# fanzhongyi/ExploreMultiModal

Hardware: AMD Instinct MI355X
Metric: image-text pairs/sec fwd+bwd, VLMo-Base, 1/2/4/8 MI355X; % bf16 MFMA roofline (higher is better)
Workload: dtype bf16

## Files before the change

### exploremultimodal_amd/csrc/attention.hip

```cpp
#include "common.h"
#include "vlmo_hip.h"

namespace {

struct AttnArgs {
    const bf16* qkv;
    const bf16* ctx;
    const bf16* dctx;
    bf16* out;
    float* lse;
    float* qvsum;
    const int32_t* seg;
    const int32_t* keymask;
    int lse_stride, heads, d;
    float scale, scale_log2e;
    uint32_t drop_thresh, drop_cmp;
    float inv_keep;
    uint64_t seed;
    int bh0;
};

#define LOG2E 1.4426950408889634f
#define LN2 0.6931471805599453f

// ... 216 lines not shown
    const bool active = w < nq;
    const int qi = w * 32 + l31;
    const int qrow = sr.row(qi);
    bf16x8 qf[4];
    if (active) {
        const bf16* qp = a.qkv + (size_t)qrow * ld + hd * 64 + 8 * h;
#pragma unroll
        for (int s = 0; s < 4; ++s) qf[s] = *(const bf16x8*)(qp + 16 * s);
    }
    const int ninstr = FRINGE ? min(nq * 4, NPAD >> 3) : nq * 4;
    for (int ii = w; ii < ninstr; ii += nw) {
        const int chhi = lane >> 5, rowlo = (lane >> 2) & 7, pc = lane & 3;
        const int row = ii * 8 + rowlo;
        const int ch = chhi * 4 + (pc ^ ((row >> 2) & 3));
        const size_t r = (size_t)sr.row(row);
        glds16(a.qkv + r * ld + a.d + hd * 64 + ch * 8, Kimg + ii * 1024);
        glds16(a.qkv + r * ld + 2 * a.d + hd * 64 + ch * 8, Vimg + ii * 1024);
    }
    if (FRINGE && nq == 9 && w < 4) {
        const int chhi = lane >> 5, rowlo = (lane >> 2) & 7, pc = lane & 3;
        const int row = w * 8 + rowlo;
        const int ch = chhi * 4 + (pc ^ ((row >> 2) & 3));
        glds16(a.qkv + (size_t)sr.row(256 + row) * ld + hd * 64 + ch * 8, Pbuf + w * 1024);
    }
    for (int i = threadIdx.x; i < (FRINGE ? 288 : NPAD); i += blockDim.x) {
        kbias[i] = key_bias(a.keymask, sr.row(i), i, N);
    }
    asm volatile("s_waitcnt vmcnt(0)" ::: "memory");
    __syncthreads();
    if (!active) return;

    const int xq = (l31 >> 2) & 3;
    const int rf0 = 1024 * (l31 >> 3) + 64 * (l31 & 7) + 16 * (h ^ xq);
    const int rf1 = 1024 * (l31 >> 3) + 64 * (l31 & 7) + 16 * ((2 + h) ^ xq);
    const int tg = (lane >> 4) & 1, tq = (lane >> 2) & 3, tp = lane & 3;
    const int trl = 64 * (4 * h + tq) + 16 * ((2 * tg + (tp >> 1)) ^ h) + 8 * (tp & 1);
    const int trh = 1024 + 64 * (4 * h + tq) + 16 * ((2 * tg + (tp >> 1)) ^ ((2 + h) & 3)) + 8 * (tp & 1);
    auto rfrag = [&](const char* img_rb, int s) -> bf16x8 {
        return *(const bf16x8*)(img_rb + 512 * (s >> 1) + ((s & 1) ? rf1 : rf0));
    };
    auto tfrag = [&](const char* img_rb, int dt) -> bf16x8 {
        const bf16x4 lo = lds_tr4<bf16>(img_rb + 512 * dt + trl);
        const bf16x4 hi = lds_tr4<bf16>(img_rb + 512 * dt + trh);
        return bf16x8{lo[0], lo[1], lo[2], lo[3], hi[0], hi[1], hi[2], hi[3]};
    };
    auto other_half = [&](float v) -> float {
        const uint32_t u = __builtin_bit_cast(uint32_t, v);
        const auto r = __builtin_amdgcn_permlane32_swap(u, u, false, false);
        return __builtin_bit_cast(float, h ? r[0] : r[1]);
    };
    auto s_tile = [&](int kt) -> f32x16 {
        f32x16 acc;
        const float* kb = kbias + kt * 32 + 4 * h;
#pragma unroll
        for (int g4 = 0; g4 < 4; ++g4) {
            const f32x4 v = *(const f32x4*)(kb + 8 * g4);
#pragma unroll
            for (int e = 0; e < 4; ++e) acc[4 * g4 + e] = v[e];
        }
        const char* kimg = Kimg + 4096 * kt;
#pragma unroll
        for (int s = 0; s < 4; ++s) acc = Elem<bf16>::mfma(rfrag(kimg, s), qf[s], acc);
        return acc;
    };

    const uint32_t akey = att_key(a.seed, bh + a.bh0);
    const uint32_t rq = ((uint32_t)qi * 512u + 4u * h) * ATT_G + akey;
    const float c2 = a.scale_log2e;
    const float thr = 8.f / c2;
    float m_run = -INFINITY;
    f32x2 l2 = {0.f, 0.f};
    f32x16 O[2] = {zero16(), zero16()};
    auto consume = [&](f32x16& S, int kt) {
        float mx = fmaxf(fmaxf(S[0], S[1]), S[2]);
#pragma unroll
        for (int i = 3; i < 15; i += 2) mx = fmaxf(fmaxf(mx, S[i]), S[i + 1]);
        mx = fmaxf(mx, S[15]);
        mx = fmaxf(mx, other_half(mx));
        if (__builtin_amdgcn_ballot_w64(mx - m_run > thr)) {
            asm volatile("" ::: "memory");
            const float m_new = fmaxf(m_run, mx);
            const float alpha = (m_run == -INFINITY) ? 1.f : __builtin_amdgcn_exp2f((m_run - m_new) * c2);
            l2 *= alpha;
#pragma unroll
            for (int dt = 0; dt < 2; ++dt)
#pragma unroll
                for (int i = 0; i < 16; ++i) O[dt][i] *= alpha;
            m_run = m_new;
        }
        const float msub = (m_run == -INFINITY) ? 0.f : -m_run * c2;
        const f32x2 c2v = {c2, c2}, msv = {msub, msub};
#pragma unroll
        for (int i = 0; i < 16; i += 2) {
            const f32x2 t = f32x2{S[i], S[i + 1]} * c2v + msv;
            const f32x2 pr = {__builtin_amdgcn_exp2f(t[0]), __builtin_amdgcn_exp2f(t[1])};
            l2 += pr;
            S[i] = pr[0];
            S[i + 1] = pr[1];
        }
        if (a.drop_thresh) S = drop_tile(S, rq + (uint32_t)(kt * 32) * ATT_G, a.drop_cmp);
        const char* vimg = Vimg + 4096 * kt;
#pragma unroll
        for (int s2 = 0; s2 < 2; ++s2) {
            bf16x8 pf;
#pragma unroll
            for (int j = 0; j < 8; ++j) pf[j] = (bf16)S[8 * s2 + j];
#pragma unroll
            for (int dt = 0; dt < 2; ++dt) O[dt] = Elem<bf16>::mfma(tfrag(vimg + 2048 * s2, dt), pf, O[dt]);
        }
    };
    f32x16 S0 = s_tile(0), S1;
    for (int kt = 0; kt < nq; kt += 2) {
        if (kt + 1 < nq) S1 = s_tile(kt + 1);
        __builtin_amdgcn_sched_barrier(0);
        consume(S0, kt);
        __builtin_amdgcn_sched_barrier(0);
        if (kt + 1 < nq) {
            if (kt + 2 < nq) S0 = s_tile(kt + 2);
            __builtin_amdgcn_sched_barrier(0);
            consume(S1, kt + 1);
            __builtin_amdgcn_sched_barrier(0);
        }
    }
    const float l_run = l2[0] + l2[1];
    const float l_tot = l_run + other_half(l_run);
    if (qi < N) store_ctx(a, O, l_tot, (m_run * c2 + log2f(l_tot)) * LN2, bh, hd, qi, qrow, h);

    if constexpr (FRINGE) {
        if (nq < 9) return;
        float* fmax = kbias + 288;
        float* fsum = fmax + 288;
        bf16x8 qF[4];
#pragma unroll
        for (int s = 0; s < 4; ++s) qF[s] = rfrag(Pbuf, s);
        auto s_fringe = [&](int kt) -> f32x16 {
            f32x16 acc;
            const float* kb = kbias + kt * 32 + 4 * h;
#pragma unroll
            for (int g4 = 0; g4 < 4; ++g4) {
                const f32x4 v = *(const f32x4*)(kb + 8 * g4);
#pragma unroll
                for (int e = 0; e < 4; ++e) acc[4 * g4 + e] = v[e];
            }
            const char* kimg = Kimg + 4096 * kt;
#pragma unroll
            for (int s = 0; s < 4; ++s) acc = Elem<bf16>::mfma(rfrag(kimg, s), qF[s], acc);
            return acc;
        };
        auto tile_max = [&](const f32x16& S) -> float {
            float mx = S[0];
#pragma unroll
            for (int i = 1; i < 16; ++i) mx = fmaxf(mx, S[i]);
            return fmaxf(mx, other_half(mx));
        };
        const bool two = (w == 0);
        f32x16 SA = s_fringe(w), SB = SA;
        if (two) SB = s_fringe(8);
        {
            const float ma = tile_max(SA), mb = tile_max(SB);
            if (h == 0) {
                fmax[w * 32 + l31] = ma;
                if (two) fmax[8 * 32 + l31] = mb;
            }
        }
        __syncthreads();
        float mstar = fmax[l31];
#pragma unroll
        for (int t = 1; t < 9; ++t) mstar = fmaxf(mstar, fmax[t * 32 + l31]);
        const float msubF = (mstar == -INFINITY) ? 0.f : -mstar * c2;
        const uint32_t rqF = ((uint32_t)(256 + l31) * 512u + 4u * h) * ATT_G + akey;
        auto soft_pack = [&](f32x16& S, int kt, bf16x8 (&pf)[2]) {
            float l = 0.f;
#pragma unroll
            for (int i = 0; i < 16; ++i) {
                S[i] = __builtin_amdgcn_exp2f(fmaf(S[i], c2, msubF));
                l += S[i];
            }
            l += other_half(l);
            if (h == 0) fsum[kt * 32 + l31] = l;
            if (a.drop_thresh) S = drop_tile(S, rqF + (uint32_t)(kt * 32) * ATT_G, a.drop_cmp);
#pragma unroll
            for (int s2 = 0; s2 < 2; ++s2)
#pragma unroll
                for (int j = 0; j < 8; ++j) pf[s2][j] = (bf16)S[8 * s2 + j];
        };
        bf16x8 pA[2], pB[2];
        soft_pack(SA, w, pA);
        if (two) soft_pack(SB, 8, pB);
        const int dtF = w & 1;
        f32x16 OF = zero16();
        for (int g = 0; g < 3; ++g) {
            if (w / 3 == g) {
                *(bf16x8*)(Pbuf + (w % 3) * 2048 + lane * 16) = pA[0];
                *(bf16x8*)(Pbuf + (w % 3) * 2048 + 1024 + lane * 16) = pA[1];
            }
            if (g == 2 && two) {
                *(bf16x8*)(Pbuf + 2 * 2048 + lane * 16) = pB[0];
                *(bf16x8*)(Pbuf + 2 * 2048 + 1024 + lane * 16) = pB[1];
            }
            __syncthreads();
            if (w >= 6) {
#pragma unroll
                for (int j = 0; j < 3; ++j)
#pragma unroll
                    for (int s2 = 0; s2 < 2; ++s2) {
                        const bf16x8 pf = *(const bf16x8*)(Pbuf + j * 2048 + s2 * 1024 + lane * 16);
                        OF = Elem<bf16>::mfma(tfrag(Vimg + 4096 * (3 * g + j) + 2048 * s2, dtF), pf, OF);
                    }
            }
            if (g < 2) __syncthreads();
        }
        const int qiF = 256 + l31;
        if (w >= 6 && qiF < N) {
            float l = fsum[l31];
#pragma unroll
            for (int t = 1; t < 9; ++t) l += fsum[t * 32 + l31];
            const float inv = a.inv_keep / l;
            bf16* op = a.out + (size_t)sr.row(qiF) * a.d + hd * 64 + 4 * h + dtF * 32;
#pragma unroll
            for (int g4 = 0; g4 < 4; ++g4) {
                bf16x4 o = {(bf16)(OF[4 * g4 + 0] * inv), (bf16)(OF[4 * g4 + 1] * inv), (bf16)(OF[4 * g4 + 2] * inv),
                            (bf16)(OF[4 * g4 + 3] * inv)};
                *(bf16x4*)(op + 8 * g4) = o;
            }
            if (w == 6 && h == 0 && a.lse) a.lse[(size_t)bh * a.lse_stride + qiF] = (mstar * c2 + log2f(l)) * LN2;
        }
    }
}

__device__ __forceinline__ float half_wave_total(float v) {
    float s_ = v + dpp_mov<0x111, 0xf, 0xf>(v);
    s_ += dpp_mov<0x112, 0xf, 0xf>(v);
    s_ += dpp_mov<0x113, 0xf, 0xf>(v);
    s_ += dpp_mov<0x114, 0xf, 0xe>(s_);
    s_ += dpp_mov<0x118, 0xf, 0xc>(s_);
    s_ += dpp_mov<0x142, 0xa, 0xf>(s_);
    return s_;
}
__device__ __forceinline__ void colsum_tile(const f32x16& t, float w, float scale, float* acc, int lane) {
    const int h = lane >> 5;
#pragma unroll
    for (int r = 0; r < 16; ++r) {
        const float v = half_wave_total(t[r] * w);
        if ((lane & 31) == 31) atomicAdd(acc + (r & 3) + 8 * (r >> 2) + 4 * h, v * scale);
    }
}
__device__ __forceinline__ void colsum_tiles(const f32x16* t, float w, float scale, float* acc, int lane) {
#pragma unroll
    for (int dt = 0; dt < 2; ++dt) colsum_tile(t[dt], w, scale, acc + dt * 32, lane);
}

__device__ __forceinline__ int slot_off(int k, int q) {
    return k * 64 + ((((q >> 2) ^ (k >> 1)) & 7) << 3) + (q & 3) * 2;
}
template <bool FRINGE>
__global__ __launch_bounds__(512) void attn_bwd1_kernel(const AttnArgs a, const int NPAD) {
    const int IMG = NPAD * 128;
    extern __shared__ __attribute__((aligned(16))) char smem[];
    char* Qimg = smem;
    char* Dimg = smem + IMG;
    char* Kimg = smem + 2 * IMG;
    const int nt = NPAD >> 5;
    char* slots = smem + 3 * IMG;
    float* kbias = (float*)(slots + 2 * nt * 2048);
    float* nlq = kbias + NPAD;
    float* ndl = nlq + NPAD;
    float* csum = ndl + NPAD;
    char* V8img = (char*)(csum + 128);

    const int lane = threadIdx.x & 63;
    const int w = __builtin_amdgcn_readfirstlane(threadIdx.x >> 6);
    const int nw = blockDim.x >> 6;
    const int bh = blockIdx.x, sidx = bh / a.heads, hd = bh % a.heads;
    const int ld = 3 * a.d;
    const SeqRows sr(a.seg, sidx);
    const int N = sr.N;
    const int nq = (N + 31) >> 5;
    const int nc = FRINGE ? min(nq, 8) : nq;
    for (int ii = w; ii < nq * 4; ii += nw) {
        const int chhi = lane >> 5, rowlo = (lane >> 2) & 7, pc = lane & 3;
        const int row = ii * 8 + rowlo;
        const int ch = chhi * 4 + (pc ^ ((row >> 2) & 3));
        const size_t r = (size_t)sr.row(row);
        glds16(a.qkv + r * ld + hd * 64 + ch * 8, Qimg + ii * 1024);
        glds16(a.qkv + r * ld + a.d + hd * 64 + ch * 8, Kimg + ii * 1024);
        glds16(a.dctx + r * a.d + hd * 64 + ch * 8, Dimg + ii * 1024);
    }
    if (FRINGE && nq > 8 && w >= 4) {
        const int chhi = lane >> 5, rowlo = (lane >> 2) & 7, pc = lane & 3;
        const int row = 256 + (w - 4) * 8 + rowlo;
        const int ch = chhi * 4 + (pc ^ ((row >> 2) & 3));
        glds16(a.qkv + (size_t)sr.row(row) * ld + 2 * a.d + hd * 64 + ch * 8, V8img + (w - 4) * 1024);
    }
    const int l31 = lane & 31, h = lane >> 5;
    const bool active = w < nc;
    const int ki = w * 32 + l31;
    const int krow = sr.row(ki);
    bf16x8 vf[4];
    if (active) {
        const bf16* kp = a.qkv + (size_t)krow * ld + a.d + hd * 64 + 8 * h;
#pragma unroll
        for (int s = 0; s < 4; ++s) vf[s] = *(const bf16x8*)(kp + a.d + 16 * s);
    }
    for (int i = threadIdx.x; i < 128; i += blockDim.x) csum[i] = 0.f;
    const float keep_prob = 1.f / a.inv_keep;
    const float inv_scale = 1.f / a.scale;
    for (int i = threadIdx.x; i < NPAD; i += blockDim.x) {
        float dl = 0.f, lq = INFINITY;
        const int row = sr.row(i);
        const float kb = key_bias(a.keymask, row, i, N);
        if (i < N) {
            const size_t o = (size_t)row * a.d + hd * 64;
            bf16x8 x[8], y[8];
#pragma unroll
            for (int c = 0; c < 8; ++c) {
                x[c] = *(const bf16x8*)(a.ctx + o + 8 * c);
                y[c] = *(const bf16x8*)(a.dctx + o + 8 * c);
            }
            lq = a.lse[(size_t)bh * a.lse_stride + i];
#pragma unroll
            for (int c = 0; c < 8; ++c)
#pragma unroll
                for (int j = 0; j < 8; ++j) dl += (float)x[c][j] * (float)y[c][j];
        }
        kbias[i] = kb;
        ndl[i] = -dl * keep_prob;
        nlq[i] = -lq * inv_scale;
    }
    asm volatile("s_waitcnt vmcnt(0)" ::: "memory");
    __syncthreads();

    const uint32_t akey = att_key(a.seed, bh + a.bh0);
    const float out_scale = a.scale * a.inv_keep;
    const float c_l2 = a.scale_log2e;
    const float kb_own = kbias[min(ki, NPAD - 1)];
    const uint32_t rl_own = (uint32_t)ki * ATT_G + akey + (uint32_t)(4 * h) * ATT_G512;
    f32x16 dK[2] = {zero16(), zero16()}, dV[2] = {zero16(), zero16()}, dQ[2] = {zero16(), zero16()};

    const int xq = (l31 >> 2) & 3;
    const int rf0 = 1024 * (l31 >> 3) + 64 * (l31 & 7) + 16 * (h ^ xq);
    const int rf1 = 1024 * (l31 >> 3) + 64 * (l31 & 7) + 16 * ((2 + h) ^ xq);
    const int tg = (lane >> 4) & 1, tq = (lane >> 2) & 3, tp = lane & 3;
    const int trl = 64 * (4 * h + tq) + 16 * ((2 * tg + (tp >> 1)) ^ h) + 8 * (tp & 1);
    const int trh = 1024 + 64 * (4 * h + tq) + 16 * ((2 * tg + (tp >> 1)) ^ ((2 + h) & 3)) + 8 * (tp & 1);
    auto rfrag = [&](const char* img_rb, int s) __attribute__((always_inline)) -> bf16x8 {
        return *(const bf16x8*)(img_rb + 512 * (s >> 1) + ((s & 1) ? rf1 : rf0));
    };
    auto tfrag = [&](const char* img_rb, int dt) __attribute__((always_inline)) -> bf16x8 {
        const bf16x4 lo = lds_tr4<bf16>(img_rb + 512 * dt + trl);
        const bf16x4 hi = lds_tr4<bf16>(img_rb + 512 * dt + trh);
        return bf16x8{lo[0], lo[1], lo[2], lo[3], hi[0], hi[1], hi[2], hi[3]};
    };
    const int sw0 = slot_off(l31, 4 * h), sw1 = slot_off(l31, 8 + 4 * h);
    const int srl = slot_off(4 * h + tq, 16 * tg + 4 * tp), srh = slot_off(8 + 4 * h + tq, 16 * tg + 4 * tp);
    auto sfrag = [&](const char* slot, int s2) __attribute__((always_inline)) -> bf16x8 {
        const bf16x4 lo = lds_tr4<bf16>(slot + 1024 * s2 + srl);
        const bf16x4 hi = lds_tr4<bf16>(slot + 1024 * s2 + srh);
        return bf16x8{lo[0], lo[1], lo[2], lo[3], hi[0], hi[1], hi[2], hi[3]};
    };

    bf16x8 qa[4], da[4], pf[2], sf[2];
    f32x16 S, dP;
    auto fetch_a = [&](int qt_) __attribute__((always_inline)) {
#pragma unroll
        for (int s = 0; s < 4; ++s) {
            qa[s] = rfrag(Qimg + qt_ * 4096, s);
            da[s] = rfrag(Dimg + qt_ * 4096, s);
        }
    };
    auto qtile = [&](int t_) __attribute__((always_inline)) {
        int q_ = w + t_;
        return q_ >= nc ? q_ - nc : q_;
    };
    auto stage_sdp = [&](int qt, const char* ktile, const bf16x8 (&vfr)[4]) __attribute__((always_inline)) {
        dP = zero16();
#pragma unroll
        for (int g4 = 0; g4 < 4; ++g4) {
            const f32x4 l4 = *(const f32x4*)(nlq + qt * 32 + 8 * g4 + 4 * h);
#pragma unroll
            for (int e = 0; e < 4; ++e) S[4 * g4 + e] = l4[e];
        }
#pragma unroll
        for (int s = 0; s < 4; ++s) {
            S = Elem<bf16>::mfma(qa[s], rfrag(ktile, s), S);
            dP = Elem<bf16>::mfma(da[s], vfr[s], dP);
        }
        __builtin_amdgcn_sched_barrier(0);
    };
    auto stage_valu_dvdk = [&](int qt, char* myslot, float kb, uint32_t rl, f32x16 (&dV)[2],
                               f32x16 (&dK)[2]) __attribute__((always_inline)) {
        bf16x8 dtr[2], qtr[2];
#pragma unroll
        for (int dt = 0; dt < 2; ++dt) {
            dtr[dt] = tfrag(Dimg + qt * 4096, dt);
            qtr[dt] = tfrag(Qimg + qt * 4096, dt);
        }
        __builtin_amdgcn_sched_barrier(0);
        if (a.drop_thresh) {
            const uint32_t rqt = rl + (uint32_t)(qt * 32) * ATT_G512;
#pragma unroll
            for (int g4 = 0; g4 < 4; ++g4) {
                const f32x4 nd = *(const f32x4*)(ndl + qt * 32 + 8 * g4 + 4 * h);
#pragma unroll
                for (int e = 0; e < 4; ++e) {
                    const int i = 4 * g4 + e;
                    const float p = __builtin_amdgcn_exp2f(fmaf(S[i], c_l2, kb));
                    const bool keep = att_mix(rqt + (uint32_t)(8 * g4 + e) * ATT_G512) >= a.drop_cmp;
                    const float pd = keep ? p : 0.f;
                    pf[i >> 3][i & 7] = (bf16)pd;
                    sf[i >> 3][i & 7] = (bf16)fmaf(pd, dP[i], p * nd[e]);
                }
            }
        } else {
#pragma unroll
            for (int g4 = 0; g4 < 4; ++g4) {
                const f32x4 nd = *(const f32x4*)(ndl + qt * 32 + 8 * g4 + 4 * h);
#pragma unroll
                for (int e = 0; e < 4; ++e) {
                    const int i = 4 * g4 + e;
                    const float p = __builtin_amdgcn_exp2f(fmaf(S[i], c_l2, kb));
                    pf[i >> 3][i & 7] = (bf16)p;
                    sf[i >> 3][i & 7] = (bf16)(p * (dP[i] + nd[e]));
                }
            }
        }
#pragma unroll
        for (int s2 = 0; s2 < 2; ++s2) {
            *(bf16x4*)(myslot + (sw0 ^ (32 * s2))) = bf16x4{sf[s2][0], sf[s2][1], sf[s2][2], sf[s2][3]};
            *(bf16x4*)(myslot + (sw1 ^ (32 * s2))) = bf16x4{sf[s2][4], sf[s2][5], sf[s2][6], sf[s2][7]};
        }
        __builtin_amdgcn_sched_barrier(0);
        bf16x8 dtr1[2], qtr1[2];
#pragma unroll
        for (int dt = 0; dt < 2; ++dt) {
            dtr1[dt] = tfrag(Dimg + qt * 4096 + 2048, dt);
            qtr1[dt] = tfrag(Qimg + qt * 4096 + 2048, dt);
        }
#pragma unroll
        for (int dt = 0; dt < 2; ++dt) {
            dV[dt] = Elem<bf16>::mfma(dtr[dt], pf[0], dV[dt]);
            dK[dt] = Elem<bf16>::mfma(qtr[dt], sf[0], dK[dt]);
        }
#pragma unroll
        for (int dt = 0; dt < 2; ++dt) {
            dV[dt] = Elem<bf16>::mfma(dtr1[dt], pf[1], dV[dt]);
            dK[dt] = Elem<bf16>::mfma(qtr1[dt], sf[1], dK[dt]);
        }
        __builtin_amdgcn_sched_barrier(0);
    };
    auto stage_dq_at = [&](const char* slot, const char* ktile, int next_q) __attribute__((always_inline)) {
        bf16x8 ktr[2][2], sb[2];
#pragma unroll
        for (int s2 = 0; s2 < 2; ++s2) {
            sb[s2] = sfrag(slot, s2);
#pragma unroll
            for (int dt = 0; dt < 2; ++dt) ktr[s2][dt] = tfrag(ktile + 2048 * s2, dt);
        }
        if (next_q >= 0) fetch_a(next_q);
        __builtin_amdgcn_sched_barrier(0);
#pragma unroll
        for (int s2 = 0; s2 < 2; ++s2)
#pragma unroll
            for (int dt = 0; dt < 2; ++dt) dQ[dt] = Elem<bf16>::mfma(ktr[s2][dt], sb[s2], dQ[dt]);
        __builtin_amdgcn_sched_barrier(0);
    };
    auto stage_dq = [&](int t, int next_q) __attribute__((always_inline)) {
        int wp = w - t;
        if (wp < 0) wp += nc;
        stage_dq_at(slots + ((t & 1) * nt + wp) * 2048, Kimg + wp * 4096, next_q);
    };
    const char* kown = Kimg + w * 4096;
    auto core_sdp = [&](int qt) __attribute__((always_inline)) { stage_sdp(qt, kown, vf); };
    auto core_valu_dvdk = [&](int qt, int t) __attribute__((always_inline)) {
        stage_valu_dvdk(qt, slots + ((t & 1) * nt + w) * 2048, kb_own, rl_own, dV, dK);
    };
    if (w >= 4) __builtin_amdgcn_s_setprio(1);
    if (!active) {
        for (int t = 0; t < nc; ++t) __syncthreads();
    } else if (w < 4) {
        fetch_a(w);
        for (int t = 0; t < nc; ++t) {
            const int qt = qtile(t);
            core_sdp(qt);
            core_valu_dvdk(qt, t);
            __syncthreads();
            stage_dq(t, t + 1 < nc ? qtile(t + 1) : -1);
        }
    } else {
        fetch_a(w);
        core_sdp(w);
        for (int t = 0; t < nc; ++t) {
            core_valu_dvdk(qtile(t), t);
            if (t > 0) stage_dq(t - 1, -1);
            if (t + 1 < nc) {
                fetch_a(qtile(t + 1));
                core_sdp(qtile(t + 1));
            }
            __syncthreads();
        }
        stage_dq(nc - 1, -1);
    }
    if (FRINGE && nq > 8) {
        auto store_tile = [&](const f32x16 (&t)[2], float sc, int row, int col0) __attribute__((always_inline)) {
            bf16* op = a.out + (size_t)row * ld + col0 + hd * 64 + 4 * h;
#pragma unroll
            for (int dt = 0; dt < 2; ++dt)
#pragma unroll
                for (int g4 = 0; g4 < 4; ++g4)
                    *(bf16x4*)(op + dt * 32 + 8 * g4) =
                        bf16x4{(bf16)(t[dt][4 * g4 + 0] * sc), (bf16)(t[dt][4 * g4 + 1] * sc),
                               (bf16)(t[dt][4 * g4 + 2] * sc), (bf16)(t[dt][4 * g4 + 3] * sc)};
        };
        fetch_a(8);
        stage_sdp(8, kown, vf);
        stage_valu_dvdk(8, slots + w * 2048, kb_own, rl_own, dV, dK);
        store_tile(dK, out_scale, krow, a.d);
        store_tile(dV, a.inv_keep, krow, 2 * a.d);
        if (a.qvsum) colsum_tiles(dV, 1.f, a.inv_keep, csum + 64, lane);
        dK[0] = zero16(), dK[1] = zero16(), dV[0] = zero16(), dV[1] = zero16();
        __syncthreads();
        const int k8 = 256 + l31;
        const char* k8tile = Kimg + 8 * 4096;
        const float kb8 = kbias[k8];
        const uint32_t rl8 = (uint32_t)k8 * ATT_G + akey + (uint32_t)(4 * h) * ATT_G512;
#pragma unroll
        for (int s = 0; s < 4; ++s) vf[s] = rfrag(V8img, s);
        char* slot1 = slots + (nt + w) * 2048;
        fetch_a(w);
        stage_sdp(w, k8tile, vf);
        stage_valu_dvdk(w, slot1, kb8, rl8, dV, dK);
        stage_dq_at(slot1, k8tile, w == 0 ? 8 : -1);
        if (w == 0) {
            stage_sdp(8, k8tile, vf);
            stage_valu_dvdk(8, slots + 8 * 2048, kb8, rl8, dV, dK);
        }
        store_tile(dQ, out_scale, krow, 0);
        if (a.qvsum) colsum_tiles(dQ, 1.f, out_scale, csum, lane);
        __syncthreads();
        auto put = [&](int region) __attribute__((always_inline)) {
            f32x4* p = (f32x4*)(smem + region * 16384) + lane;
#pragma unroll
            for (int dt = 0; dt < 2; ++dt)
#pragma unroll
                for (int g4 = 0; g4 < 4; ++g4) {
                    p[(dt * 4 + g4) * 64] = f32x4{dK[dt][4 * g4], dK[dt][4 * g4 + 1], dK[dt][4 * g4 + 2], dK[dt][4 * g4 + 3]};
                    p[(8 + dt * 4 + g4) * 64] = f32x4{dV[dt][4 * g4], dV[dt][4 * g4 + 1], dV[dt][4 * g4 + 2], dV[dt][4 * g4 + 3]};
                }
        };
        auto add = [&](int region) __attribute__((always_inline)) {
            const f32x4* p = (const f32x4*)(smem + region * 16384) + lane;
#pragma unroll
            for (int dt = 0; dt < 2; ++dt)
#pragma unroll
                for (int g4 = 0; g4 < 4; ++g4) {
                    const f32x4 uk = p[(dt * 4 + g4) * 64], uv = p[(8 + dt * 4 + g4) * 64];
#pragma unroll
                    for (int e = 0; e < 4; ++e) dK[dt][4 * g4 + e] += uk[e], dV[dt][4 * g4 + e] += uv[e];
                }
        };
        const int row8 = sr.row(k8);
        const float wt8 = k8 < N ? 1.f : 0.f;
        if (w >= 4) put(w - 4);
        if (w == 4 || w == 5) {
            const int dt = w - 4;
            f32x16 acc = zero16();
            for (int k = 0; k < 9; ++k) {
                const char* slot = slots + k * 2048;
                const bf16x8 s0 = sfrag(slot, 0), s1 = sfrag(slot, 1);
                const bf16x8 k0 = tfrag(Kimg + k * 4096, dt), k1 = tfrag(Kimg + k * 4096 + 2048, dt);
                acc = Elem<bf16>::mfma(k0, s0, acc);
                acc = Elem<bf16>::mfma(k1, s1, acc);
            }
            if (k8 < N) {
                bf16* op = a.out + (size_t)row8 * ld + hd * 64 + dt * 32 + 4 * h;
#pragma unroll
                for (int g4 = 0; g4 < 4; ++g4)
                    *(bf16x4*)(op + 8 * g4) =
                        bf16x4{(bf16)(acc[4 * g4 + 0] * out_scale), (bf16)(acc[4 * g4 + 1] * out_scale),
                               (bf16)(acc[4 * g4 + 2] * out_scale), (bf16)(acc[4 * g4 + 3] * out_scale)};
            }
            if (a.qvsum) colsum_tile(acc, wt8, out_scale, csum + dt * 32, lane);
        }
        __syncthreads();
        if (w < 4) add(w);
        if (w >= 1 && w < 4) put(w);
        __syncthreads();
        if (w == 0) {
            add(1), add(2), add(3);
            if (k8 < N) {
                store_tile(dK, out_scale, row8, a.d);
                store_tile(dV, a.inv_keep, row8, 2 * a.d);
            }
            if (a.qvsum) colsum_tiles(dV, wt8, a.inv_keep, csum + 64, lane);
        }
    } else if (active && ki < N) {
        bf16* op = a.out + (size_t)krow * ld + hd * 64 + 4 * h;
#pragma unroll
        for (int dt = 0; dt < 2; ++dt)
#pragma unroll
            for (int g4 = 0; g4 < 4; ++g4) {
                bf16x4 oq = {(bf16)(dQ[dt][4 * g4 + 0] * out_scale), (bf16)(dQ[dt][4 * g4 + 1] * out_scale),
                             (bf16)(dQ[dt][4 * g4 + 2] * out_scale), (bf16)(dQ[dt][4 * g4 + 3] * out_scale)};
                bf16x4 ok = {(bf16)(dK[dt][4 * g4 + 0] * out_scale), (bf16)(dK[dt][4 * g4 + 1] * out_scale),
                             (bf16)(dK[dt][4 * g4 + 2] * out_scale), (bf16)(dK[dt][4 * g4 + 3] * out_scale)};
                bf16x4 ov = {(bf16)(dV[dt][4 * g4 + 0] * a.inv_keep), (bf16)(dV[dt][4 * g4 + 1] * a.inv_keep),
                             (bf16)(dV[dt][4 * g4 + 2] * a.inv_keep), (bf16)(dV[dt][4 * g4 + 3] * a.inv_keep)};
                *(bf16x4*)(op + dt * 32 + 8 * g4) = oq;
                *(bf16x4*)(op + a.d + dt * 32 + 8 * g4) = ok;
                *(bf16x4*)(op + 2 * a.d + dt * 32 + 8 * g4) = ov;
            }
    }
    if (a.qvsum) {
        if (active && !(FRINGE && nq > 8)) {
            const float wt = ki < N ? 1.f : 0.f;
            colsum_tiles(dQ, wt, out_scale, csum, lane);
            colsum_tiles(dV, wt, a.inv_keep, csum + 64, lane);
        }
        __syncthreads();
        for (int i = threadIdx.x; i < 128; i += blockDim.x) {
            float* dst = a.qvsum + (size_t)sidx * 2 * a.d + (i >> 6) * a.d + hd * 64 + (i & 63);
            *dst = csum[i];
        }
    }
}

#define ATT_LW 8
#define ATT_LCH 4
#define ATT_LBUF (ATT_LCH * 4096)
#define ATT_LMAX 1024
#define ATT_LDS_FWD (4 * ATT_LBUF + ATT_LMAX * 4)
#define ATT_LDS_BWD (4 * ATT_LBUF + 3 * ATT_LMAX * 4 + ATT_LW * 64 * 4)

__device__ __forceinline__ uint32_t att_stride(int N) { return N > 512 ? 1024u : 512u; }

__device__ __forceinline__ void stage_chunk(const bf16* pa, int lda, const bf16* pb, int ldb, const SeqRows& sr, int t0,
                                            int nt, char* ia, char* ib, int w, int lane) {
    const int chhi = lane >> 5, rowlo = (lane >> 2) & 7, pc = lane & 3;
    for (int ii = w; ii < nt * 4; ii += ATT_LW) {
        const int row = t0 * 32 + ii * 8 + rowlo;
        const int ch = chhi * 4 + (pc ^ ((row >> 2) & 3));
        const size_t r = (size_t)sr.row(row);
        glds16(pa + r * lda + ch * 8, ia + ii * 1024);
        glds16(pb + r * ldb + ch * 8, ib + ii * 1024);
    }
}

__device__ __forceinline__ void colsum_wave(const f32x16* t, float wt, float* part, int lane) {
    const int h = lane >> 5;
#pragma unroll
    for (int dt = 0; dt < 2; ++dt)
#pragma unroll
        for (int r = 0; r < 16; ++r) {
            const float v = half_wave_total(t[dt][r] * wt);
            if ((lane & 31) == 31) part[dt * 32 + (r & 3) + 8 * (r >> 2) + 4 * h] += v;
        }
}

__device__ __forceinline__ void bwd_row_constants(const AttnArgs& a, const SeqRows& sr, int bh, int hd, int npad,
                                                  float* lseq, float* delta, float* kbias) {
    const float keep_prob = 1.f / a.inv_keep;
    for (int i = threadIdx.x; i < npad; i += blockDim.x) {
        float dl = 0.f, lq = INFINITY;
        const int row = sr.row(i);
        if (i < sr.N) {
            const size_t o = (size_t)row * a.d + hd * 64;
            bf16x8 x[8], y[8];
#pragma unroll
            for (int c = 0; c < 8; ++c) {
                x[c] = *(const bf16x8*)(a.ctx + o + 8 * c);
                y[c] = *(const bf16x8*)(a.dctx + o + 8 * c);
            }
            lq = a.lse[(size_t)bh * a.lse_stride + i] * LOG2E;
#pragma unroll
            for (int c = 0; c < 8; ++c)
#pragma unroll
                for (int j = 0; j < 8; ++j) dl += (float)x[c][j] * (float)y[c][j];
        }
        delta[i] = dl * keep_prob;
        lseq[i] = lq;
        if (kbias) kbias[i] = key_bias(a.keymask, row, i, sr.N);
    }
}

__global__ __launch_bounds__(512) void attn_fwd_long_kernel(const AttnArgs a) {
    extern __shared__ __attribute__((aligned(16))) char smem[];
    char* ring = smem;
    float* kbias = (float*)(smem + 4 * ATT_LBUF);

    const int lane = threadIdx.x & 63;
    const int w = __builtin_amdgcn_readfirstlane(threadIdx.x >> 6);
    const int bh = blockIdx.x, sidx = bh / a.heads, hd = bh % a.heads;
    const int ld = 3 * a.d;
    const SeqRows sr(a.seg, sidx);
    const int N = sr.N;
    if (N <= 0) return;
    const int nq = (N + 31) >> 5, nch = (nq + ATT_LCH - 1) / ATT_LCH, nrounds = (nq + ATT_LW - 1) / ATT_LW;
    const bf16* kb0 = a.qkv + a.d + hd * 64;
    const bf16* vb0 = a.qkv + 2 * a.d + hd * 64;
    stage_chunk(kb0, ld, vb0, ld, sr, 0, min(ATT_LCH, nq), ring, ring + ATT_LBUF, w, lane);
    for (int i = threadIdx.x; i < nq * 32; i += blockDim.x) kbias[i] = key_bias(a.keymask, sr.row(i), i, N);

    const int l31 = lane & 31, h = lane >> 5;
    const uint32_t akey = att_key(a.seed, bh + a.bh0);
    const uint32_t stride = att_stride(N);
    int qi = 0, qrow = 0;
    uint32_t rq = 0;
    bf16x8 qf[4];
    float m_run = -INFINITY, l_run = 0.f;
    f32x16 O[2] = {zero16(), zero16()};
    const int nsteps = nrounds * nch;
    for (int j = 0; j < nsteps; ++j) {
        const int rd = j / nch, c = j - rd * nch;
        asm volatile("s_waitcnt vmcnt(0)" ::: "memory");
        __syncthreads();
        if (j + 1 < nsteps) {
            const int t0 = ((j + 1) % nch) * ATT_LCH;
            char* nb = ring + ((j + 1) & 1) * 2 * ATT_LBUF;
            stage_chunk(kb0, ld, vb0, ld, sr, t0, min(ATT_LCH, nq - t0), nb, nb + ATT_LBUF, w, lane);
        }
        const char* Kc = ring + (j & 1) * 2 * ATT_LBUF;
        const char* Vc = Kc + ATT_LBUF;
        const int qt = rd * ATT_LW + w;
        if (qt >= nq) continue;
        if (c == 0) {
            qi = qt * 32 + l31;
            qrow = sr.row(qi);
            rq = ((uint32_t)qi * stride + 4u * h) * ATT_G + akey;
            const bf16* qp = a.qkv + (size_t)qrow * ld + hd * 64 + 8 * h;
#pragma unroll
            for (int s = 0; s < 4; ++s) qf[s] = *(const bf16x8*)(qp + 16 * s);
            m_run = -INFINITY, l_run = 0.f;
            O[0] = zero16(), O[1] = zero16();
        }
        const int c0 = c * ATT_LCH;
        f32x16 S[ATT_LCH];
        float mx = -INFINITY;
#pragma unroll
        for (int cc = 0; cc < ATT_LCH; ++cc) {
            S[cc] = zero16();
            const int kt = c0 + cc;
            if (kt < nq) {
#pragma unroll
                for (int s = 0; s < 4; ++s) S[cc] = Elem<bf16>::mfma(row_frag(Kc, cc * 32, s, lane), qf[s], S[cc]);
#pragma unroll
                for (int g4 = 0; g4 < 4; ++g4) {
                    const f32x4 kb = *(const f32x4*)(kbias + kt * 32 + 8 * g4 + 4 * h);
#pragma unroll
                    for (int e = 0; e < 4; ++e) {
                        const float t = S[cc][4 * g4 + e] * a.scale_log2e + kb[e];
                        S[cc][4 * g4 + e] = t;
                        mx = fmaxf(mx, t);
                    }
                }
            }
        }
        mx = fmaxf(mx, __shfl_xor(mx, 32, 64));
        const float m_new = fmaxf(m_run, mx);
        const bool dead = (m_new == -INFINITY);
        const float alpha = dead ? 1.f : __builtin_amdgcn_exp2f(m_run - m_new);
        float lsum = 0.f;
#pragma unroll
        for (int cc = 0; cc < ATT_LCH; ++cc) {
            if (c0 + cc < nq) {
#pragma unroll
                for (int i = 0; i < 16; ++i) {
                    const float p = dead ? 0.f : __builtin_amdgcn_exp2f(S[cc][i] - m_new);
                    S[cc][i] = p;
                    lsum += p;
                }
            }
        }
        lsum += __shfl_xor(lsum, 32, 64);
        l_run = l_run * alpha + lsum;
        m_run = m_new;
#pragma unroll
        for (int dt = 0; dt < 2; ++dt)
#pragma unroll
            for (int i = 0; i < 16; ++i) O[dt][i] *= alpha;
#pragma unroll
        for (int cc = 0; cc < ATT_LCH; ++cc) {
            const int kt = c0 + cc;
            if (kt < nq) {
                if (a.drop_thresh) S[cc] = drop_tile(S[cc], rq + (uint32_t)(kt * 32) * ATT_G, a.drop_cmp);
#pragma unroll
                for (int s2 = 0; s2 < 2; ++s2) {
                    bf16x8 pf;
#pragma unroll
                    for (int jj = 0; jj < 8; ++jj) pf[jj] = (bf16)S[cc][8 * s2 + jj];
#pragma unroll
                    for (int dt = 0; dt < 2; ++dt)
                        O[dt] = Elem<bf16>::mfma(tr_frag(Vc, cc * 32 + 16 * s2, dt * 32, lane), pf, O[dt]);
                }
            }
// ... 577 lines not shown
```

Baseline: 4685.

## Compute attention-backward delta from LDS-staged dO with wave-parallel DPP reduction

The per-row delta term (rowsum of O·dO) was computed one row per thread, with each thread re-reading full ctx and dctx rows from global memory. Now each wave prefetches ctx fragments into registers and reads dO from the LDS image that is already staged. It reduces the dot products across 8 lanes with DPP moves, one 8-row group per wave. Because ndl is now written after the barrier, an extra __syncthreads is added before first use in both wave-role branches, with a matching extra barrier for idle waves. This costs one more block-wide sync and adds register pressure from the prefetched fragments.

```diff
diff --git a/exploremultimodal_amd/csrc/attention.hip b/exploremultimodal_amd/csrc/attention.hip
--- a/exploremultimodal_amd/csrc/attention.hip
+++ b/exploremultimodal_amd/csrc/attention.hip
@@ -542,33 +542,40 @@
 #pragma unroll
         for (int s = 0; s < 4; ++s) vf[s] = *(const bf16x8*)(kp + a.d + 16 * s);
     }
+    constexpr int NDG = FRINGE ? 5 : 4;
+    const int ndg = (N + 7) >> 3;
+    const int drow = lane >> 3, dch = lane & 7;
+    bf16x8 cx[NDG] = {};
+#pragma unroll
+    for (int g = 0; g < NDG; ++g) {
+        const int ii = w + g * nw;
+        if (ii < ndg) cx[g] = *(const bf16x8*)(a.ctx + (size_t)sr.row(ii * 8 + drow) * a.d + hd * 64 + dch * 8);
+    }
     for (int i = threadIdx.x; i < 128; i += blockDim.x) csum[i] = 0.f;
     const float keep_prob = 1.f / a.inv_keep;
     const float inv_scale = 1.f / a.scale;
     for (int i = threadIdx.x; i < NPAD; i += blockDim.x) {
-        float dl = 0.f, lq = INFINITY;
-        const int row = sr.row(i);
-        const float kb = key_bias(a.keymask, row, i, N);
-        if (i < N) {
-            const size_t o = (size_t)row * a.d + hd * 64;
-            bf16x8 x[8], y[8];
-#pragma unroll
-            for (int c = 0; c < 8; ++c) {
-                x[c] = *(const bf16x8*)(a.ctx + o + 8 * c);
-                y[c] = *(const bf16x8*)(a.dctx + o + 8 * c);
-            }
-            lq = a.lse[(size_t)bh * a.lse_stride + i];
-#pragma unroll
-            for (int c = 0; c < 8; ++c)
-#pragma unroll
-                for (int j = 0; j < 8; ++j) dl += (float)x[c][j] * (float)y[c][j];
-        }
-        kbias[i] = kb;
-        ndl[i] = -dl * keep_prob;
-        nlq[i] = -lq * inv_scale;
+        kbias[i] = key_bias(a.keymask, sr.row(i), i, N);
+        nlq[i] = -(i < N ? a.lse[(size_t)bh * a.lse_stride + i] : INFINITY) * inv_scale;
+        if (i >= N) ndl[i] = 0.f;
     }
     asm volatile("s_waitcnt vmcnt(0)" ::: "memory");
     __syncthreads();
+#pragma unroll
+    for (int g = 0; g < NDG; ++g) {
+        const int ii = w + g * nw;
+        if (ii < ndg) {
+            const bf16x8 y = *(const bf16x8*)(Dimg + att_off(ii * 8 + drow, dch));
+            float dl = 0.f;
+#pragma unroll
+            for (int j = 0; j < 8; ++j) dl += (float)cx[g][j] * (float)y[j];
+            dl += dpp_mov<0xB1, 0xf, 0xf>(dl);
+            dl += dpp_mov<0x4E, 0xf, 0xf>(dl);
+            dl += dpp_mov<0x141, 0xf, 0xf>(dl);
+            const int i = ii * 8 + drow;
+            if (dch == 0 && i < N) ndl[i] = -dl * keep_prob;
+        }
+    }
 
     const uint32_t akey = att_key(a.seed, bh + a.bh0);
     const float out_scale = a.scale * a.inv_keep;
@@ -716,12 +723,13 @@
     };
     if (w >= 4) __builtin_amdgcn_s_setprio(1);
     if (!active) {
-        for (int t = 0; t < nc; ++t) __syncthreads();
+        for (int t = 0; t <= nc; ++t) __syncthreads();
     } else if (w < 4) {
         fetch_a(w);
         for (int t = 0; t < nc; ++t) {
             const int qt = qtile(t);
             core_sdp(qt);
+            if (t == 0) __syncthreads();
             core_valu_dvdk(qt, t);
             __syncthreads();
             stage_dq(t, t + 1 < nc ? qtile(t + 1) : -1);
@@ -729,6 +737,7 @@
     } else {
         fetch_a(w);
         core_sdp(w);
+        __syncthreads();
         for (int t = 0; t < nc; ++t) {
             core_valu_dvdk(qtile(t), t);
             if (t > 0) stage_dq(t - 1, -1);
```

New measurement: 4695, median of 6. No clear change (+0.2%).
